# carlosnatalino/optical-rl-gym

Measured on NVIDIA B200. Metric: env_steps_per_sec, higher is better.
Workload: dtype u32

## Files before the change

### optical-rl-gym_b200/csrc/orlg_api.cu

```cuda
#include <atomic>
#include <cmath>
#include <condition_variable>
#include <cstdio>
#include <cstdlib>
#include <chrono>
#include <cstring>
#include <emmintrin.h>
#include <functional>
#include <memory>
#include <mutex>
#include <string>
#include <thread>
#include <vector>

#include "orlg_deeprmsa_fast.cuh"
#include "orlg_rollout.cuh"
#include "orlg_policy.cuh"
#include "orlg_step_wide.cuh"
#include "orlg_wrappers.cuh"

using namespace orlg;

static thread_local std::string g_err;

// ... 364 lines not shown
    p.seed = cfg->seed; p.env_id_base = cfg->env_id_base;
    p.mean_holding = cfg->mean_holding; p.mean_iat = cfg->mean_iat;
    p.obs_dim = cfg->kind == ORLG_DEEPRMSA ? 1 + 2 * p.N + (2 * J + 3) * p.k : 0;
    p.node_top_step = 1;
    while (p.node_top_step * 2 <= p.N - 1) p.node_top_step *= 2;
    p.cand_stride = ((p.k * J + 7) / 8) * 8;
    p.nwv = wide ? (p.S + 127) / 128 : 1;
    p.wstride = wide ? (p.nwv == 3 ? 4 : p.nwv) : 0;
    env->km = p.k <= 5 ? 5 : KMAX;
    env->obs_smem = (size_t)STEP_THREADS * p.obs_dim * (p.obs_f64 ? 8 : 4);
    if (env->obs_smem > 200 * 1024) { delete env; return fail(ORLG_E_UNSUPPORTED, "observation too large for the staging tile"); }

    int cap = cfg->heap_capacity;
    if (cap <= 0) {
        double load = cfg->mean_holding / cfg->mean_iat;
        double want = load + 8.0 * std::sqrt(load) + 16.0;
        double hard = cfg->kind == ORLG_RWA ? (double)p.E * p.S * C : (double)p.E * p.S * C / 2.0;
        cap = (int)std::ceil(want < hard ? want : hard);
    }
    cap = ((cap + EV_GROUP - 1) / EV_GROUP) * EV_GROUP;
    if (cfg->heap_capacity > 256 * EV_GROUP) {
        delete env;
        return fail(ORLG_E_UNSUPPORTED, "heap_capacity above 4096 live services per environment");
    }
    if (cap > 256 * EV_GROUP) cap = 256 * EV_GROUP;
    p.ev_groups = ((cap / EV_GROUP + 15) / 16) * 16;
    p.heap_cap = cap;

    int rc = ORLG_OK;
    const int NN = p.N * p.N, P = t->num_paths;
    std::vector<int> pair_first(t->pair_first, t->pair_first + NN);
    std::vector<unsigned char> pair_count(NN);
    for (int i = 0; i < NN; i++) pair_count[i] = (unsigned char)(t->pair_count[i] < 0 ? 0 : (t->pair_count[i] > p.k ? p.k : t->pair_count[i]));
    std::vector<unsigned> linkmask(P), meta(P);
    int se_max = 1;
    for (int r = 0; r < P; r++) {
        unsigned lm = 0;
        for (int h = t->path_link_ptr[r]; h < t->path_link_ptr[r + 1]; h++) {
            if (t->path_links[h] < 0 || t->path_links[h] >= p.E) { delete env; return fail(ORLG_E_INVALID, "path link index out of range"); }
            if (!wide) lm |= 1u << t->path_links[h];
        }
        if (t->path_hops[r] > 255 || t->path_link_ptr[r + 1] - t->path_link_ptr[r] != t->path_hops[r]) { delete env; return fail(ORLG_E_INVALID, "inconsistent path hop counts"); }
        linkmask[r] = lm;
        int se = t->path_se[r] < 1 ? 1 : t->path_se[r];
        meta[r] = (unsigned)(t->path_hops[r] & 0xff) | ((unsigned)(se & 0xff) << 8) | ((unsigned)(t->path_mod[r] & 0xff) << 16);
        se_max = se > se_max ? se : se_max;
    }
    std::vector<unsigned char> mod_se(t->num_mods > 0 ? t->num_mods : 1, 1);
    for (int m = 0; m < t->num_mods; m++) { mod_se[m] = (unsigned char)t->mod_se[m]; se_max = t->mod_se[m] > se_max ? t->mod_se[m] : se_max; }
    std::vector<unsigned char> nslots((size_t)(se_max + 1) * (br_max + 1), 1);
    bool slots_unrepresentable = false;
    for (int se = 1; se <= se_max; se++)
        for (int b = 0; b <= br_max; b++) {
            int n = (int)std::ceil((double)b / ((double)se * cfg->channel_width)) + 1;
            if (n > 200) {
                const bool configured = t->num_bit_rates > 0 ? false : (b >= cfg->bit_rate_lo && b <= cfg->bit_rate_hi);
                if (n <= p.S && configured) slots_unrepresentable = true;
                n = 200;
            }
            nslots[(size_t)se * (br_max + 1) + b] = (unsigned char)n;
        }
    for (int i = 0; i < t->num_bit_rates; i++)
        for (int se = 1; se <= se_max; se++) {
            const int n = (int)std::ceil((double)t->bit_rates[i] / ((double)se * cfg->channel_width)) + 1;
            if (n > 200 && n <= p.S) slots_unrepresentable = true;
        }
    if (slots_unrepresentable && cfg->kind != ORLG_RWA) {
        delete env;
        return fail(ORLG_E_UNSUPPORTED, "a request of this configuration may need 201.." + std::to_string(p.S) + " slots: at most 200 slots per service are representable");
    }
    std::vector<double> reach((size_t)(t->num_mods > 0 ? t->num_mods : 1) * (br_max + 1), 0.0);
    if (cfg->kind == ORLG_RMCSA)
        for (int m = 0; m < t->num_mods; m++)
            for (int b = 0; b <= br_max; b++)
                reach[(size_t)m * (br_max + 1) + b] = b == 0 ? 1e300 : reach_km(t->mod_osnr[m], t->mod_xt[m], t->mod_se[m], b, cfg->worst_xt);
    std::vector<double> plen(t->path_length, t->path_length + P);
    std::vector<unsigned> node_thr = thresholds(t->node_prob, p.N);
    std::vector<unsigned> br_thr = t->num_bit_rates > 0 ? thresholds(t->bit_rate_prob, t->num_bit_rates) : std::vector<unsigned>(1, 0u);
    std::vector<int> link_order(p.E);
    for (int l = 0; l < p.E; l++) link_order[l] = t->link_order ? t->link_order[l] : l;
    std::vector<int> bit_rates(t->num_bit_rates > 0 ? t->num_bit_rates : 1, 0);
    for (int i = 0; i < t->num_bit_rates; i++) bit_rates[i] = t->bit_rates[i];

    if (!rc) rc = dev_upload(env, &p.pair_first, pair_first);
    if (!rc) rc = dev_upload(env, &p.pair_count, pair_count);
    if (!rc) rc = dev_upload(env, &p.path_linkmask, linkmask);
    if (!rc) rc = dev_upload(env, &p.path_meta, meta);
    if (!rc) rc = dev_upload(env, &p.path_length, plen);
    {
        std::vector<int> lptr(t->path_link_ptr, t->path_link_ptr + P + 1);
        std::vector<unsigned short> l16(lptr[P] > 0 ? lptr[P] : 1, 0);
        for (int h = 0; h < lptr[P]; h++) l16[h] = (unsigned short)t->path_links[h];
        if (!rc) rc = dev_upload(env, &p.path_link_ptr, lptr);
        if (!rc) rc = dev_upload(env, &p.path_links16, l16);
    }
    if (!rc) rc = dev_upload(env, &p.nslots, nslots);
    if (!rc) rc = dev_upload(env, &p.mod_se, mod_se);
    if (!rc) rc = dev_upload(env, &p.reach, reach);
    if (!rc) rc = dev_upload(env, &p.node_thr, node_thr);
    if (!rc) rc = dev_upload(env, &p.br_thr, br_thr);
    if (!rc) rc = dev_upload(env, &p.bit_rates, bit_rates);
    if (!rc) rc = dev_upload(env, &p.link_order, link_order);
    env->alloc_is_state = true;
    const size_t n = (size_t)p.n;
    if (!rc) rc = dev_alloc(env, &p.masks, (size_t)C * p.E * (wide ? p.wstride : p.nwv) * n);
    if (!rc) rc = dev_alloc(env, &p.now, n);
    if (!rc) rc = dev_alloc(env, &p.cur_hold, n);
    if (!rc) rc = dev_alloc(env, &p.cur_req, n);
    if (!rc) rc = dev_alloc(env, &p.counters, 8 * n);
    if (!rc) rc = dev_alloc(env, &p.req_index, n);
    if (!rc) rc = dev_alloc(env, &p.nheap, n);
    if (!rc) rc = dev_alloc(env, &p.heap_min, n);
    if (!rc) rc = dev_alloc(env, &p.ev_time, n * (size_t)p.heap_cap, false);
    if (!rc) rc = dev_alloc(env, &p.ev_pay, n * (size_t)p.heap_cap, false);
    if (!rc) rc = dev_alloc(env, &p.ev_gmin, n * (size_t)p.ev_groups);
    if (!rc) rc = dev_alloc(env, &p.ev_tail, n);
    if (!rc) rc = dev_alloc(env, &p.cand, n * (size_t)p.cand_stride);
    if (!rc && wide && cfg->kind == ORLG_DEEPRMSA) rc = dev_alloc(env, &p.cand16, n * (size_t)p.cand_stride);
    if (!rc) rc = dev_alloc(env, &p.errors, n);
    if (!rc && cfg->kind == ORLG_RMSA && t->num_bit_rates > 0) rc = dev_alloc(env, &p.br_hist, 2 * (size_t)t->num_bit_rates * n);
    if (!rc && cfg->kind == ORLG_RWA) rc = dev_alloc(env, &p.act_hist, (size_t)(p.k + p.S + 2 * p.allow_rejection) * n);
    env->alloc_is_state = false;
    if (rc) { orlg_destroy(env); return rc; }

    env->fast = false;
    env->hot = false;
    env->ro_ok = false;
    if (!wide && cfg->kind != ORLG_RMCSA && p.k <= 5 && P <= 65535 && se_max <= 15 && !std::getenv("ORLG_FORCE_GENERIC")) {
        std::vector<unsigned char> blob;
        auto put = [&blob](const void *src, size_t bytes) {
            size_t off = (blob.size() + 15) / 16 * 16;
            blob.resize(off + bytes);
            std::memcpy(blob.data() + off, src, bytes);
            return (int)off;
        };
        std::vector<unsigned short> pf16(NN);
        for (int i = 0; i < NN; i++) pf16[i] = (unsigned short)(pair_first[i] < 0 ? 0 : pair_first[i]);
        std::vector<unsigned char> pse(P);
        for (int r = 0; r < P; r++) pse[r] = (unsigned char)((meta[r] >> 8) & 0xff);
        std::vector<unsigned char> ns128((size_t)(se_max + 1) * 128, 1);
        for (int se = 1; se <= se_max; se++)
            for (int b = 0; b < 128 && b <= br_max; b++) ns128[(size_t)se * 128 + b] = nslots[(size_t)se * (br_max + 1) + b];
        std::vector<float> pos(p.S + 1), nsl(32);
        for (int v = 0; v <= p.S; v++) pos[v] = (float)(2 * v - p.S) / (float)p.S;
        for (int v = 0; v < 32; v++) nsl[v] = (float)(2 * v - 11) / 7.0f;
        p.off_pair_first = put(pf16.data(), pf16.size() * 2);
        p.off_pair_count = put(pair_count.data(), pair_count.size());
        p.off_path_lm = put(linkmask.data(), linkmask.size() * 4);
        p.off_path_se = put(pse.data(), pse.size());
        std::vector<unsigned long long> pll(P, 0ULL);
        bool ll_ok = true;
        for (int r = 0; r < P; r++) {
            const int h0 = t->path_link_ptr[r], hn = t->path_link_ptr[r + 1] - h0;
            if (hn > 12) { ll_ok = false; break; }
            unsigned long long v = (unsigned long long)hn << 60;
            for (int h = 0; h < hn; h++) v |= (unsigned long long)(t->path_links[h0 + h] & 31) << (5 * h);
            pll[r] = v;
        }
        p.off_path_ll = put(pll.data(), pll.size() * 8);
        p.off_nslots = put(ns128.data(), ns128.size());
        p.off_node_thr = put(node_thr.data(), node_thr.size() * 4);
        p.off_pos = put(pos.data(), pos.size() * 4);
        p.off_nsl = put(nsl.data(), nsl.size() * 4);
        std::vector<float> rcp4(p.S / 2 + 2, 0.0f);
        for (size_t r = 1; r < rcp4.size(); r++) rcp4[r] = 1.0f / (float)(4 * r);
        p.off_rcp4 = put(rcp4.data(), rcp4.size() * 4);
        std::vector<unsigned> dbl(17, 0u);
        for (int nn = 1; nn <= 16; nn++) {
            int len = 1;
            for (int it = 0; it < 4; it++) {
                int sh = len < nn - len ? len : nn - len;
                if (sh < 0) sh = 0;
                dbl[nn] |= (unsigned)sh << (8 * it);
                len += sh;
            }
        }
        p.off_dbl = put(dbl.data(), dbl.size() * 4);
        blob.resize((blob.size() + 127) / 128 * 128);
        if (ll_ok && blob.size() <= 24 * 1024 && blob.size() + (size_t)FAST_THREADS * 16 * 32 <= 100 * 1024) {
            std::vector<uint4> blob4(blob.size() / 16);
            std::memcpy(blob4.data(), blob.data(), blob.size());
            rc = dev_upload(env, &p.tab_blob, blob4);
            if (rc) { orlg_destroy(env); return rc; }
            p.tab_vec = (int)blob4.size();
            env->fast = cfg->kind == ORLG_DEEPRMSA;
            size_t per_thread = (size_t)p.obs_dim * (p.obs_f64 ? 8 : 4);
            if (per_thread < (size_t)p.E * 16) per_thread = (size_t)p.E * 16;
            p.warp_area_bytes = (int)((per_thread * 32 + 127) / 128 * 128);
            env->fast_smem = blob.size() + (size_t)(FAST_THREADS / 32) * p.warp_area_bytes + 8 * (FAST_THREADS / 32 + 1);
            cudaError_t ea = cudaSuccess;
            if (env->fast_smem > 48 * 1024) {
                ea = cudaFuncSetAttribute(deeprmsa_fast_kernel<22, 5, 1, false>, cudaFuncAttributeMaxDynamicSharedMemorySize, (int)env->fast_smem);
                if (ea == cudaSuccess) ea = cudaFuncSetAttribute(deeprmsa_fast_kernel<0, 5, 1, false>, cudaFuncAttributeMaxDynamicSharedMemorySize, (int)env->fast_smem);
                if (ea == cudaSuccess) ea = cudaFuncSetAttribute(deeprmsa_fast_kernel<22, 5, 1, true>, cudaFuncAttributeMaxDynamicSharedMemorySize, (int)env->fast_smem);
                if (ea == cudaSuccess) ea = cudaFuncSetAttribute(deeprmsa_fast_kernel<0, 5, 1, true>, cudaFuncAttributeMaxDynamicSharedMemorySize, (int)env->fast_smem);
                if (ea == cudaSuccess) ea = cudaFuncSetAttribute(deeprmsa_fast_kernel<22, 5, 0, false>, cudaFuncAttributeMaxDynamicSharedMemorySize, (int)env->fast_smem);
                if (ea == cudaSuccess) ea = cudaFuncSetAttribute(deeprmsa_fast_kernel<0, 5, 0, false>, cudaFuncAttributeMaxDynamicSharedMemorySize, (int)env->fast_smem);
                if (ea == cudaSuccess) ea = cudaFuncSetAttribute(deeprmsa_fast_kernel<22, 5, 0, true>, cudaFuncAttributeMaxDynamicSharedMemorySize, (int)env->fast_smem);
                if (ea == cudaSuccess) ea = cudaFuncSetAttribute(deeprmsa_fast_kernel<0, 5, 0, true>, cudaFuncAttributeMaxDynamicSharedMemorySize, (int)env->fast_smem);
            }
            if (ea == cudaSuccess && env->fast_smem > 48 * 1024) {
                ea = cudaFuncSetAttribute(deeprmsa_fast_kernel<22, 5, 1, false, true>, cudaFuncAttributeMaxDynamicSharedMemorySize, (int)env->fast_smem);
                if (ea == cudaSuccess) ea = cudaFuncSetAttribute(deeprmsa_fast_kernel<0, 5, 1, false, true>, cudaFuncAttributeMaxDynamicSharedMemorySize, (int)env->fast_smem);
            }
            if (ea != cudaSuccess) env->fast = false;
            int n_hi = 0;
            for (int se = 1; se <= se_max; se++)
                for (int b = 0; b <= cfg->bit_rate_hi && b <= br_max; b++)
                    n_hi = nslots[(size_t)se * (br_max + 1) + b] > n_hi ? nslots[(size_t)se * (br_max + 1) + b] : n_hi;
            env->hot = env->fast && J == 1 && p.k == 5 && p.cand_stride == 8 && t->num_bit_rates == 0 && cfg->bit_rate_hi < 128 &&
                       cfg->bit_rate_lo >= 0 && n_hi <= 16 && (p.obs_dim & 1) == 0 && p.E <= 256 && !std::getenv("ORLG_NO_HOT");
            if (env->hot && !encode_mask_map(env)) env->hot = false;
            const bool small_n = t->num_bit_rates == 0 && cfg->bit_rate_hi < 128 && cfg->bit_rate_lo >= 0 && n_hi <= 16;
            env->ro_ok = cfg->kind == ORLG_DEEPRMSA ? env->hot
                         : (ea == cudaSuccess && p.E <= 32 && (cfg->kind == ORLG_RWA || small_n) && !std::getenv("ORLG_NO_HOT"));
        }
    }

    if (env->obs_smem > 48 * 1024) {
        cudaError_t e1 = cudaFuncSetAttribute(step_kernel<ORLG_DEEPRMSA, 5>, cudaFuncAttributeMaxDynamicSharedMemorySize, (int)env->obs_smem);
        cudaError_t e2 = cudaFuncSetAttribute(step_kernel<ORLG_DEEPRMSA, KMAX>, cudaFuncAttributeMaxDynamicSharedMemorySize, (int)env->obs_smem);
        if (e1 != cudaSuccess || e2 != cudaSuccess) { orlg_destroy(env); return fail(ORLG_E_CUDA, "cudaFuncSetAttribute(shared memory) failed"); }
    }
    *out = env;
    return ORLG_OK;
}

int orlg_destroy(orlg_env *env) {
    if (!env) return ORLG_OK;
    DeviceGuard guard(env->device);
    for (void *ptr : env->allocs) cudaFree(ptr);
    for (int i = 0; i < RO_HOST_BUFFERS; i++) {
        if (env->ro_pk_dev[i]) cudaFree(env->ro_pk_dev[i]);
        if (env->ro_pk_host[i]) cudaFreeHost(env->ro_pk_host[i]);
        if (env->ro_pk_ev[i]) cudaEventDestroy(env->ro_pk_ev[i]);
        if (env->ro_k_ev[i]) cudaEventDestroy(env->ro_k_ev[i]);
        if (env->ro_act_dev[i]) cudaFree(env->ro_act_dev[i]);
        if (env->ro_obs_dev[i]) cudaFree(env->ro_obs_dev[i]);
        if (env->ro_cp_ev[i]) cudaEventDestroy(env->ro_cp_ev[i]);
    }
    if (env->ro_copy_stream) cudaStreamDestroy(env->ro_copy_stream);
    delete env;
    return ORLG_OK;
}

int orlg_action_dim(const orlg_env *env) { return env->p.kind == ORLG_DEEPRMSA ? 1 : (env->p.kind == ORLG_RMCSA ? 4 : 2); }
int orlg_obs_dim(const orlg_env *env) { return env->p.obs_dim; }
int orlg_mask_words(const orlg_env *env) { return NW * env->p.nwv; }
int orlg_heap_capacity(const orlg_env *env) { return env->p.heap_cap; }
int64_t orlg_state_bytes(const orlg_env *env) { return env->state_bytes; }

int orlg_kernel_info(const orlg_env *env, orlg_kernel_info_t *out) {
    if (!env || !out) return fail(ORLG_E_INVALID, "null handle or output");
    out->wide = env->wide;
    out->fast = env->fast;
    out->hot = env->hot;
    out->rollout_kernel = env->ro_ok;
    out->rollout_lanes = rollout_lpw(env);
    out->link_template = !env->wide && env->p.E == 22 ? 22 : 0;
    out->last_rollout_persistent = env->ro_last_persistent;
    return ORLG_OK;
}

int orlg_seed(orlg_env *env, uint64_t seed) {
    if (!env) return fail(ORLG_E_INVALID, "null handle");
    env->p.seed = seed;
    env->cfg.seed = seed;
    return ORLG_OK;
}

int orlg_set_trace(orlg_env *env, const orlg_request *trace_dev, int64_t trace_len) {
    if (!env || (trace_len > 0 && !trace_dev)) return fail(ORLG_E_INVALID, "null trace");
    if (trace_len >= (1LL << 32)) return fail(ORLG_E_UNSUPPORTED, "trace too long");
    env->p.trace = trace_dev;
    env->p.trace_len = trace_len;
    env->p.traffic = ORLG_TRAFFIC_TRACE;
    return ORLG_OK;
}

int orlg_reset(orlg_env *env, int full, void *obs_dev, orlg_stream stream) {
    if (!env) return fail(ORLG_E_INVALID, "null handle");
    DeviceGuard guard(env->device);
    if (env->p.traffic == ORLG_TRAFFIC_TRACE && env->p.trace == nullptr) return fail(ORLG_E_INVALID, "trace traffic selected but orlg_set_trace was not called");
    StepIO io;
    std::memset(&io, 0, sizeof(io));
    io.policy = -1;
    io.obs = env->p.obs_dim ? obs_dev : nullptr;
    if (full) env->ro_valid = false;
    else {
        int rc0 = ensure_canonical(env, (cudaStream_t)stream);
        if (rc0) return rc0;
    }
    if (full) {
        fill_events_kernel<<<592, 256, 0, (cudaStream_t)stream>>>(env->p);
        CUDA_OK(cudaGetLastError());
    }
    int rc = launch_step(env, io, full ? MODE_FULL_RESET : MODE_EPISODE_RESET, (cudaStream_t)stream);
    if (rc == ORLG_OK && full) env->p.lockstep_ridx = 1;
    return rc;
}

static int step_impl(orlg_env *env, const int32_t *actions_dev, int fused_policy, int32_t *actions_out, void *obs_dev, float *reward_dev,
                     uint8_t *done_dev, int32_t *decision_dev, int64_t *info_dev, orlg_stream stream) {
    {
        int rc0 = ensure_canonical(env, (cudaStream_t)stream);
        if (rc0) return rc0;
    }
    StepIO io;
    io.policy = fused_policy;
// ... 861 lines not shown
```

### optical-rl-gym_b200/csrc/orlg_rollout.cuh

```cuda
#pragma once
#include "orlg_deeprmsa_fast.cuh"

#ifndef ORLG_RO_BULK
#define ORLG_RO_BULK 1
#endif

namespace orlg {

constexpr int RO_WCAP = 64;
#ifndef ORLG_RO_SIDE
#define ORLG_RO_SIDE 4
#endif
constexpr int RO_SIDE = ORLG_RO_SIDE;
constexpr int RO_MAX_THREADS = 448;
enum { RO_POLICY_RANDOM = 0, RO_POLICY_SP_FF = 1, RO_POLICY_SAP_FF = 2, RO_POLICY_REPLAY = 3, RO_POLICY_LLP_FF = 4, RO_POLICY_SAP_LF = 5 };

#ifdef ORLG_PHASE_TIMING
#define RPH_INIT() long long rph_t_ = clock64()
#define RPH_MARK(k)                                                                                      \
    do {                                                                                                 \
        long long rph_n_ = clock64();                                                                    \
        if ((threadIdx.x & 31) == 0) atomicAdd(&g_phase_cycles[k], (unsigned long long)(rph_n_ - rph_t_)); \
        rph_t_ = rph_n_;                                                                                 \
    } while (0)
// ... 439 lines not shown
                if (POLICY == RO_POLICY_SP_FF) {
                    if (npaths_cur > 0 && (candw & 0xffu) != CAND_NONE) { act = 0; act_slot = (int)(candw & 0xffu); }
                } else if (POLICY == RO_POLICY_LLP_FF) {
                    int best = KIND == ORLG_RWA ? -1 : 0;
                    for (int q = 0; q < npaths_cur; q++) {
                        const unsigned st = (unsigned)((candw >> (8 * q)) & 0xffu);
                        const int fr = (int)((candt >> (8 * q)) & 0xffu);
                        if (st != CAND_NONE && fr > best) { best = fr; act = q; act_slot = (int)st; }
                    }
                } else if (KIND == ORLG_RWA) {
                    int best_hops = 0x7fffffff;
                    for (int q = 0; q < npaths_cur; q++) {
                        const unsigned st = (unsigned)((candw >> (8 * q)) & 0xffu);
                        const int hops = (int)((candh >> (4 * q)) & 0xfu);
                        if (hops < best_hops && st != CAND_NONE) { best_hops = hops; act = q; act_slot = (int)st; }
                    }
                } else {
                    for (int q = npaths_cur - 1; q >= 0; q--) {
                        const unsigned st = (unsigned)((candw >> (8 * q)) & 0xffu);
                        if (st != CAND_NONE) { act = q; act_slot = (int)st; }
                    }
                }
            }
            if (POLICY != RO_POLICY_REPLAY && ra.actions) {
                if (KIND == ORLG_DEEPRMSA) ra.actions[(size_t)t * p.n + env] = act;
                else *reinterpret_cast<int2 *>(ra.actions + ((size_t)t * p.n + env) * 2) = make_int2(act, act_slot);
            }

            bool accepted = false;
            int a_start = 0;
            if (KIND == ORLG_RWA && p.act_hist) {
                const int R = p.k + p.allow_rejection, Cn = p.S + p.allow_rejection;
                if (act >= 0 && act < R && act_slot >= 0 && act_slot < Cn) {
                    atomicAdd(p.act_hist + (size_t)act * p.n + env, 1);
                    atomicAdd(p.act_hist + (size_t)(R + act_slot) * p.n + env, 1);
                } else {
                    err |= ORLG_ERR_NO_SUCH_PATH;
                }
            }
            if (act >= 0 && act < p.k && (KIND == ORLG_DEEPRMSA || (act_slot >= 0 && act_slot < p.S))) {
                if (act < np_cur) {
                    const int a_row = s_pair_first[pair] + act;
                    const int a_n = KIND == ORLG_RWA ? 1 : s_nslots[s_path_se[a_row] * 128 + br];
                    const unsigned a_lm = s_path_lm[a_row];
                    bool fits;
                    if (KIND == ORLG_DEEPRMSA) {
                        const unsigned st = (unsigned)((candw >> (8 * act)) & 0xffu);
                        fits = st != CAND_NONE;
                        a_start = (int)st;
                    } else if (checked) {
                        fits = true; a_start = act_slot;
                    } else {
                        a_start = act_slot;
                        fits = a_start + a_n <= p.S;
                        if (fits) {
                            Bits F = bits_ones();
                            unsigned m = a_lm;
                            while (m) {
                                const int l = __ffs(m) - 1;
                                m &= m - 1;
                                F = bits_and(F, bits_from(sm[l * 32]));
                            }
                            fits = bits_contains(F, bits_range_short(a_start, a_n));
                        }
                    }
                    if (fits) {
                        if (nlive + 1 > (unsigned)p.heap_cap) {
                            err |= ORLG_ERR_HEAP_OVERFLOW;
                        } else {
                            ro_path_update<false>(sm, a_lm, bits_range_short(a_start, a_n));
                            const double rel = __dadd_rn(now, hold);
                            const unsigned long long pl = pack_service(a_row, a_start, a_n, 0, sid);
                            bool in_side = false;
                            if (rel <= hzn) {
#pragma unroll
                                for (int s = 0; s < RO_SIDE; s++) {
                                    if (!in_side && !(side_t[s * 32] < ORLG_INF)) {
                                        side_t[s * 32] = rel; side_p[s * 32] = pl; in_side = true;
                                    }
                                }
                                if (in_side) side_min = dmin(side_min, rel);
                            }
                            if (!in_side) {
                                win_store(ev + n_tab * 32, rel, pl); n_tab++;
                                tmin_tab = dmin(tmin_tab, rel);
                            }
                            nlive++;
                            d_acc += 1; ep_acc += 1;
                            if (KIND != ORLG_RWA) { d_prov += br; ep_prov += br; }
                            accepted = true;
                        }
                    }
                } else {
                    err |= ORLG_ERR_NO_SUCH_PATH;
                }
            }
            if (KIND == ORLG_RWA) { d_proc += 1; ep_proc += 1; }
            if (ra.reward) ra.reward[(size_t)t * p.n + env] = accepted ? 1.0f : (KIND == ORLG_DEEPRMSA ? -1.0f : 0.0f);
            rec_flags = ((unsigned)act & 0xffffu) | (accepted ? (1u << 28) : 0u);

            RPH_MARK(1);
            now = TRACE ? t_arrival : __dadd_rn(now, e_iat);
            hold = e_hold; src = p_src; dst = p_dst; br = p_br;
            ridx++;
            sid = ep_proc;
            if (KIND != ORLG_RWA) { d_proc += 1; ep_proc += 1; d_req += br; ep_req += br; }
            npaths_cur = npaths;
            RO_POP_DUE();
            if (side_min <= now) {
                double m2 = ORLG_INF;
#pragma unroll
                for (int s = 0; s < RO_SIDE; s++) {
                    const double ts = side_t[s * 32];
                    if (ts <= now) {
                        const unsigned long long pl = side_p[s * 32];
                        const int rs = svc_start(pl);
                        ro_path_update<true>(sm, s_path_lm[svc_row(pl)], bits_range_short(rs, svc_slots(pl)));
                        side_t[s * 32] = ORLG_INF;
                        nlive--;
                    } else {
                        m2 = dmin(m2, ts);
                    }
                }
                side_min = m2;
            }
        }
        RPH_MARK(2);
        for (int tries = 0; t >= 0 && __any_sync(0xffffffffu, live && tmin_tab <= now); tries++) {
            RPH_COUNT(15);
            hzn = tries < 60 ? __dadd_rn(now, __dmul_rn(ra.span, __longlong_as_double((long long)(1023 - tries) << 52))) : now;
            RTL_REBUILD_BEGIN();
            unsigned long long g_rtl_scan_ = 0, g_rtl_sort_ = 0;
            ro_rebuild(ev, (unsigned)p.heap_cap, side_t, side_p, n_tab, wh, wn, tmin_tab, side_min, hzn, head, nxt, lane, g_rtl_scan_, g_rtl_sort_);
            RO_POP_DUE();
            RTL_REBUILD_END();
        }
        RPH_MARK(3);
        if (live && t >= 0) {
            done = (ep_proc == p.episode_length);
            if (done && p.auto_reset) {
                ep_acc = 0; ep_prov = 0;
                if (KIND == ORLG_RWA) { ep_proc = 0; ep_req = 0; } else { ep_proc = 1; ep_req = br; }
            }
            if (ra.done) ra.done[(size_t)t * p.n + env] = done ? 1 : 0;
        }

        unsigned feat[KM];
#pragma unroll
        for (int q = 0; q < KM; q++) feat[q] = 0;
        if (live) {
            unsigned long long cand_out = 0xFFFFFFFFFFFFFFFFULL, tot_out = 0;
            unsigned hops_out = 0;
            const int first = s_pair_first[src * p.N + dst];
#pragma unroll 1
            for (int q = 0; q < KM; q++) {
                const bool have = q < npaths;
                const int row = have ? first + q : first;
                unsigned lm = have ? s_path_lm[row] : 0u;
                Bits A = have ? bits_ones() : Bits{{0u, 0u, 0u, 0u}};
                while (lm) {
                    const int l0 = __ffs(lm) - 1;
                    lm &= lm - 1;
                    const int l1 = lm ? __ffs(lm) - 1 : l0;
                    lm &= lm - 1;
                    const int l2 = lm ? __ffs(lm) - 1 : l0;
                    lm &= lm - 1;
                    const int l3 = lm ? __ffs(lm) - 1 : l0;
                    lm &= lm - 1;
                    const uint4 v0 = sm[l0 * 32], v1 = sm[l1 * 32], v2 = sm[l2 * 32], v3 = sm[l3 * 32];
                    A.w[0] &= v0.x & v1.x; A.w[1] &= v0.y & v1.y; A.w[2] &= v0.z & v1.z; A.w[3] &= v0.w & v1.w;
                    A.w[0] &= v2.x & v3.x; A.w[1] &= v2.y & v3.y; A.w[2] &= v2.z & v3.z; A.w[3] &= v2.w & v3.w;
                }
                int st;
                unsigned f = 0;
                if (KIND == ORLG_DEEPRMSA) {
                    const int n = s_nslots[s_path_se[row] * 128 + br];
                    const Bits B = bits_runs_ge_sched(A, s_dbl[n]);
                    st = bits_ffs_flat(B);
                    const int fe = bits_ffs_flat(bits_andnot(B, bits_shr1(B)));
                    const int total = bits_popc(A);
                    const int runs = bits_popc(bits_andnot(A, bits_shl1(A)));
                    f = feat_pack(st, fe - st + n, total, runs, n);
                } else {
                    if (KIND == ORLG_RWA) {
                        if (POLICY == RO_POLICY_SAP_LF) { Bits L = A; L.w[0] &= ~1u; st = bits_fls(L); }
                        else st = bits_ffs_flat(A);
                        if (have) hops_out |= (unsigned)(s_path_ll[row] >> 60) << (4 * q);
                    } else {
                        const int n = s_nslots[s_path_se[row] * 128 + br];
                        const Bits B = bits_and(bits_runs_ge_sched(A, s_dbl[n]), bits_range(0, max(p.S - n, 0)));
                        st = bits_ffs_flat(B);
                    }
                    tot_out |= (unsigned long long)(bits_popc(A) & 0xff) << (8 * q);
                }
                cand_out = st >= 0 ? ((cand_out & ~(0xFFULL << (8 * q))) | ((unsigned long long)st << (8 * q))) : cand_out;
#pragma unroll
                for (int i = 0; i < KM; i++) feat[i] = i == q ? f : feat[i];
            }
            if (KIND != ORLG_DEEPRMSA) { candt = tot_out; candh = hops_out; }
            candw = cand_out;
        }
        RPH_MARK(5);
        if (t < 0) continue;
        if (KIND == ORLG_DEEPRMSA && ra.packed && live) {
            uint4 *rec = ra.packed + ((size_t)t * p.n + env) * 2;
            rec[0] = make_uint4(feat[0], feat[1], feat[2], feat[3]);
            rec[1] = make_uint4(feat[4], (unsigned)br | ((unsigned)src << 8) | ((unsigned)dst << 16) | ((unsigned)npaths << 24) |
                                             (rec_flags & (1u << 28)) | (done ? (1u << 29) : 0u),
                                rec_flags & 0xffffu, 0u);
        }
        if (KIND == ORLG_DEEPRMSA && ra.obs) {
            const unsigned tile = ro_tile_acquire(pool_free, lane);
            unsigned char *stage = pool + (size_t)tile * ra.tile_bytes;
            RPH_MARK(4);
            if (live) {
                float *so32 = reinterpret_cast<float *>(stage) + (size_t)lane * p.obs_dim;
                float2 *r2 = reinterpret_cast<float2 *>(so32);
                const int lo_n = min(src, dst), hi_n = max(src, dst);
                for (int q = 0; q < p.N; q++) r2[q] = make_float2(0.0f, 0.0f);
                float v[2 + 5 * KM];
                v[0] = hi_n == p.N - 1 ? 1.0f : 0.0f;
                v[1 + 5 * KM] = 0.0f;
#pragma unroll
                for (int q = 0; q < KM; q++) {
                    const unsigned f = feat[q];
                    const int st = (int)(f & 127u), len = (int)((f >> 7) & 127u), total = (int)((f >> 14) & 127u);
                    const int runs = (int)((f >> 21) & 63u), n = (int)(f >> 27);
                    const bool have = q < npaths, blk = st != 127;
                    v[1 + 5 * q] = blk ? s_pos[blk ? st : 0] : -1.0f;
                    v[2 + 5 * q] = blk ? (float)(len - 8) * 0.125f : -1.0f;
                    v[3 + 5 * q] = have ? s_nsl[n] : -1.0f;
                    v[4 + 5 * q] = have ? s_pos[total] : -1.0f;
                    v[5 + 5 * q] = runs > 0 ? (float)(total - 4 * runs) * s_rcp4[runs] : -1.0f;
                }
#pragma unroll
                for (int i = 0; i < (1 + 5 * KM + 1) / 2; i++) r2[p.N + i] = make_float2(v[2 * i], v[2 * i + 1]);
                so32[0] = __fdiv_rn((float)br, 100.0f);
                so32[1 + lo_n] = 1.0f;
                if (hi_n != p.N - 1) so32[1 + p.N + hi_n] = 1.0f;
            }
            RPH_MARK(6);
            {
                float *g = ra.obs + ((size_t)t * p.n + env0) * p.obs_dim;
                const int total_el = nvalid * p.obs_dim;
#if ORLG_RO_BULK
                asm volatile("fence.proxy.async.shared::cta;" ::: "memory");
                __syncwarp();
                if ((reinterpret_cast<size_t>(g) & 15) == 0 && (total_el & 3) == 0) {
                    if (lane == 0) {
                        asm volatile("cp.async.bulk.global.shared::cta.bulk_group [%0], [%1], %2;"
                                     ::"l"(g), "r"((unsigned)__cvta_generic_to_shared(stage)), "r"((unsigned)total_el * 4u) : "memory");
                        asm volatile("cp.async.bulk.commit_group;" ::: "memory");
                        asm volatile("cp.async.bulk.wait_group.read 0;" ::: "memory");
                    }
                } else {
                    const float *sv = reinterpret_cast<const float *>(stage);
                    for (int q = lane; q < total_el; q += 32) g[q] = sv[q];
                }
#else
                __syncwarp();
                if ((reinterpret_cast<size_t>(g) & 15) == 0 && (total_el & 3) == 0) {
                    const uint4 *sv = reinterpret_cast<const uint4 *>(stage);
                    uint4 *gv = reinterpret_cast<uint4 *>(g);
#pragma unroll 7
                    for (int q = lane; q < total_el / 4; q += 32) gv[q] = sv[q];
                } else {
                    const float *sv = reinterpret_cast<const float *>(stage);
                    for (int q = lane; q < total_el; q += 32) g[q] = sv[q];
                }
#endif
            }
            ro_tile_release(pool_free, tile, lane);
        }
        RPH_MARK(7);
    }
#undef RO_POP_DUE
    RTL_SET(2);

    if (live) {
        ra.st_ntab[env] = n_tab; ra.st_wh[env] = wh; ra.st_wn[env] = wn;
        ra.st_tmin[env] = tmin_tab; ra.st_hzn[env] = hzn;
#pragma unroll
        for (int s = 0; s < RO_SIDE; s++) {
            ra.st_side_t[(size_t)s * p.n + env] = side_t[s * 32];
            ra.st_side_p[(size_t)s * p.n + env] = side_p[s * 32];
        }
        uint4 *mw = p.masks + env;
        for (int l = 0; l < E; l++) mw[(size_t)l * p.n] = sm[l * 32];
        p.now[env] = now;
        p.cur_hold[env] = hold;
        p.cur_req[env] = make_uint2((unsigned)src | ((unsigned)dst << 8) | ((unsigned)br << 16), (unsigned)sid);
        {
            const auto c0 = p.counters[(size_t)0 * p.n + env], c1 = p.counters[(size_t)1 * p.n + env];
            const auto c4 = p.counters[(size_t)4 * p.n + env], c5 = p.counters[(size_t)5 * p.n + env];
            p.counters[(size_t)0 * p.n + env] = c0 + d_proc;
            p.counters[(size_t)1 * p.n + env] = c1 + d_acc;
            p.counters[(size_t)4 * p.n + env] = c4 + d_req;
            p.counters[(size_t)5 * p.n + env] = c5 + d_prov;
        }
        p.counters[(size_t)2 * p.n + env] = ep_proc;
        p.counters[(size_t)3 * p.n + env] = ep_acc;
        p.counters[(size_t)6 * p.n + env] = ep_req;
        p.counters[(size_t)7 * p.n + env] = ep_prov;
        p.req_index[env] = ridx;
        p.nheap[env] = nlive;
        p.errors[env] = err;
        if (KIND == ORLG_DEEPRMSA) *reinterpret_cast<unsigned long long *>(p.cand + (size_t)env * 8) = candw;
    }
    RPH_MARK(9);
    RTL_SET(3);
    RTL_FLUSH((unsigned)gwarp);
}

__global__ void __launch_bounds__(128) ro_canonicalize_kernel(const Params p, const RolloutArgs ra) {
    const int env = blockIdx.x * blockDim.x + threadIdx.x;
    if (env >= p.n) return;
    const int lane = env % ra.lpw;
    const size_t gw = (size_t)(env / ra.lpw);
    WinEntry *const ev = ra.ev + gw * (size_t)(p.heap_cap + 2 * RO_WCAP) * 32 + lane;
    const WinEntry *const win = ev + (size_t)(p.heap_cap + RO_WCAP) * 32;
    unsigned n_tab = ra.st_ntab[env];
    const unsigned wh = ra.st_wh[env], wn = ra.st_wn[env], n_entry = ra.st_ncanon[env];
    unsigned err = 0;
    for (unsigned j = wh; j < wn; j++) {
        const WinEntry w = win_load(win + j * 32);
        win_store(ev + n_tab * 32, w.t, w.p); n_tab++;
    }
#pragma unroll
    for (int s = 0; s < RO_SIDE; s++) {
        const double ts = ra.st_side_t[(size_t)s * p.n + env];
        if (ts < ORLG_INF) { win_store(ev + n_tab * 32, ts, ra.st_side_p[(size_t)s * p.n + env]); n_tab++; }
    }
    if (n_tab != p.nheap[env]) err |= ORLG_ERR_LOCKSTEP;
    double *ev_t = p.ev_time + (size_t)env * p.heap_cap;
    unsigned long long *ev_p = p.ev_pay + (size_t)env * p.heap_cap;
    float *gmin = p.ev_gmin + (size_t)env * p.ev_groups;
    const unsigned n_fill = max(n_tab, n_entry);
    for (unsigned s0 = 0; s0 < n_fill; s0 += 8) {
        double tt[8];
        unsigned long long pp[8];
#pragma unroll
        for (int i = 0; i < 8; i++) {
            const bool in = s0 + i < n_tab;
            WinEntry w;
            w.t = ORLG_INF; w.p = 0ULL;
            if (in) w = win_load(ev + (s0 + i) * 32);
            tt[i] = w.t; pp[i] = w.p;
        }
#pragma unroll
        for (int i = 0; i < 4; i++) {
// ... 24 lines not shown
```

Before: 5.981 billion.

## Walk packed per-path link lists instead of bitmask ffs loop; pair paths for RMSA/RWA

Candidate scoring now reads each path's links from a packed 64-bit list (hop count plus 5-bit link ids) instead of pulling links out of a 32-bit mask with repeated ffs. Host packing pads unused slots with the first link, so four-link chunks can read past the hop count without changing the AND result. The non-DeepRMSA branch handles two paths per iteration to expose more independent shared-memory loads. Risks: paths with zero hops, or more than 12, now mark the packing invalid, and the kernel branch may not check that flag. The paired loop also runs to the longer path's hop count.

Result: faster. 6.275 billion (median of 6 runs) (+4.9%).

```diff
diff --git a/optical-rl-gym_b200/csrc/orlg_api.cu b/optical-rl-gym_b200/csrc/orlg_api.cu
--- a/optical-rl-gym_b200/csrc/orlg_api.cu
+++ b/optical-rl-gym_b200/csrc/orlg_api.cu
@@ -540,9 +540,9 @@
         bool ll_ok = true;
         for (int r = 0; r < P; r++) {
             const int h0 = t->path_link_ptr[r], hn = t->path_link_ptr[r + 1] - h0;
-            if (hn > 12) { ll_ok = false; break; }
+            if (hn > 12 || hn < 1) { ll_ok = false; break; }
             unsigned long long v = (unsigned long long)hn << 60;
-            for (int h = 0; h < hn; h++) v |= (unsigned long long)(t->path_links[h0 + h] & 31) << (5 * h);
+            for (int h = 0; h < 12; h++) v |= (unsigned long long)(t->path_links[h0 + (h < hn ? h : 0)] & 31) << (5 * h);
             pll[r] = v;
         }
         p.off_path_ll = put(pll.data(), pll.size() * 8);
diff --git a/optical-rl-gym_b200/csrc/orlg_rollout.cuh b/optical-rl-gym_b200/csrc/orlg_rollout.cuh
--- a/optical-rl-gym_b200/csrc/orlg_rollout.cuh
+++ b/optical-rl-gym_b200/csrc/orlg_rollout.cuh
@@ -615,50 +615,86 @@
             unsigned long long cand_out = 0xFFFFFFFFFFFFFFFFULL, tot_out = 0;
             unsigned hops_out = 0;
             const int first = s_pair_first[src * p.N + dst];
+            if (KIND == ORLG_DEEPRMSA) {
 #pragma unroll 1
-            for (int q = 0; q < KM; q++) {
-                const bool have = q < npaths;
-                const int row = have ? first + q : first;
-                unsigned lm = have ? s_path_lm[row] : 0u;
-                Bits A = have ? bits_ones() : Bits{{0u, 0u, 0u, 0u}};
-                while (lm) {
-                    const int l0 = __ffs(lm) - 1;
-                    lm &= lm - 1;
-                    const int l1 = lm ? __ffs(lm) - 1 : l0;
-                    lm &= lm - 1;
-                    const int l2 = lm ? __ffs(lm) - 1 : l0;
-                    lm &= lm - 1;
-                    const int l3 = lm ? __ffs(lm) - 1 : l0;
-                    lm &= lm - 1;
-                    const uint4 v0 = sm[l0 * 32], v1 = sm[l1 * 32], v2 = sm[l2 * 32], v3 = sm[l3 * 32];
-                    A.w[0] &= v0.x & v1.x; A.w[1] &= v0.y & v1.y; A.w[2] &= v0.z & v1.z; A.w[3] &= v0.w & v1.w;
-                    A.w[0] &= v2.x & v3.x; A.w[1] &= v2.y & v3.y; A.w[2] &= v2.z & v3.z; A.w[3] &= v2.w & v3.w;
-                }
-                int st;
-                unsigned f = 0;
-                if (KIND == ORLG_DEEPRMSA) {
+                for (int q = 0; q < KM; q++) {
+                    const bool have = q < npaths;
+                    const int row = have ? first + q : first;
+                    unsigned long long ll = s_path_ll[row];
                     const int n = s_nslots[s_path_se[row] * 128 + br];
-                    const Bits B = bits_runs_ge_sched(A, s_dbl[n]);
-                    st = bits_ffs_flat(B);
+                    const unsigned sched = s_dbl[n];
+                    Bits A = have ? bits_ones() : Bits{{0u, 0u, 0u, 0u}};
+                    for (int h = have ? (int)(ll >> 60) : 0; h > 0; h -= 4, ll >>= 20) {
+                        const unsigned w = (unsigned)ll;
+                        const uint4 v0 = sm[(w & 31u) * 32], v1 = sm[((w >> 5) & 31u) * 32];
+                        const uint4 v2 = sm[((w >> 10) & 31u) * 32], v3 = sm[((w >> 15) & 31u) * 32];
+                        A.w[0] &= v0.x & v1.x; A.w[1] &= v0.y & v1.y; A.w[2] &= v0.z & v1.z; A.w[3] &= v0.w & v1.w;
+                        A.w[0] &= v2.x & v3.x; A.w[1] &= v2.y & v3.y; A.w[2] &= v2.z & v3.z; A.w[3] &= v2.w & v3.w;
+                    }
+                    RPH_MARK(10);
+                    const Bits B = bits_runs_ge_sched(A, sched);
+                    const int st = bits_ffs_flat(B);
                     const int fe = bits_ffs_flat(bits_andnot(B, bits_shr1(B)));
                     const int total = bits_popc(A);
                     const int runs = bits_popc(bits_andnot(A, bits_shl1(A)));
-                    f = feat_pack(st, fe - st + n, total, runs, n);
-                } else {
-                    if (KIND == ORLG_RWA) {
-                        if (POLICY == RO_POLICY_SAP_LF) { Bits L = A; L.w[0] &= ~1u; st = bits_fls(L); }
-                        else st = bits_ffs_flat(A);
-                        if (have) hops_out |= (unsigned)(s_path_ll[row] >> 60) << (4 * q);
-                    } else {
-                        const int n = s_nslots[s_path_se[row] * 128 + br];
-                        const Bits B = bits_and(bits_runs_ge_sched(A, s_dbl[n]), bits_range(0, max(p.S - n, 0)));
-                        st = bits_ffs_flat(B);
-                    }
-                    tot_out |= (unsigned long long)(bits_popc(A) & 0xff) << (8 * q);
-                }
-                cand_out = st >= 0 ? ((cand_out & ~(0xFFULL << (8 * q))) | ((unsigned long long)st << (8 * q))) : cand_out;
-#pragma unroll
-                for (int i = 0; i < KM; i++) feat[i] = i == q ? f : feat[i];
+                    const unsigned f = feat_pack(st, fe - st + n, total, runs, n);
+                    cand_out = st >= 0 ? ((cand_out & ~(0xFFULL << (8 * q))) | ((unsigned long long)st << (8 * q))) : cand_out;
+#pragma unroll
+                    for (int i = 0; i < KM; i++) feat[i] = i == q ? f : feat[i];
+                    RPH_MARK(5);
+                }
+            } else {
+#pragma unroll 1
+                for (int q = 0; q < KM; q += 2) {
+                    bool have[2];
+                    int row[2], n[2] = {0, 0};
+                    unsigned sched[2] = {0u, 0u};
+                    unsigned long long ll[2];
+                    Bits A[2];
+#pragma unroll
+                    for (int j = 0; j < 2; j++) {
+                        have[j] = q + j < npaths;
+                        row[j] = have[j] ? first + q + j : first;
+                        ll[j] = s_path_ll[row[j]];
+                        if (KIND != ORLG_RWA) {
+                            n[j] = s_nslots[s_path_se[row[j]] * 128 + br];
+                            sched[j] = s_dbl[n[j]];
+                        }
+                        A[j] = have[j] ? bits_ones() : Bits{{0u, 0u, 0u, 0u}};
+                    }
+                    const int hops = max(have[0] ? (int)(ll[0] >> 60) : 0, have[1] ? (int)(ll[1] >> 60) : 0);
+                    for (int s = 0; s < 5 * hops; s += 10) {
+                        uint4 v[2][2];
+#pragma unroll
+                        for (int j = 0; j < 2; j++)
+#pragma unroll
+                            for (int h = 0; h < 2; h++) v[j][h] = sm[(int)((ll[j] >> (s + 5 * h)) & 31u) * 32];
+#pragma unroll
+                        for (int j = 0; j < 2; j++) {
+                            A[j].w[0] &= v[j][0].x & v[j][1].x;
+                            A[j].w[1] &= v[j][0].y & v[j][1].y;
+                            A[j].w[2] &= v[j][0].z & v[j][1].z;
+                            A[j].w[3] &= v[j][0].w & v[j][1].w;
+                        }
+                    }
+                    RPH_MARK(10);
+#pragma unroll
+                    for (int j = 0; j < 2; j++) {
+                        const int qj = q + j;
+                        int st;
+                        if (KIND == ORLG_RWA) {
+                            if (POLICY == RO_POLICY_SAP_LF) { Bits L = A[j]; L.w[0] &= ~1u; st = bits_fls(L); }
+                            else st = bits_ffs_flat(A[j]);
+                            if (have[j]) hops_out |= (unsigned)(ll[j] >> 60) << (4 * qj);
+                        } else {
+                            const Bits B = bits_and(bits_runs_ge_sched(A[j], sched[j]), bits_range(0, max(p.S - n[j], 0)));
+                            st = bits_ffs_flat(B);
+                        }
+                        tot_out |= (unsigned long long)(bits_popc(A[j]) & 0xff) << (8 * qj);
+                        cand_out = st >= 0 ? ((cand_out & ~(0xFFULL << (8 * qj))) | ((unsigned long long)st << (8 * qj))) : cand_out;
+                    }
+                    RPH_MARK(5);
+                }
             }
             if (KIND != ORLG_DEEPRMSA) { candt = tot_out; candh = hops_out; }
             candw = cand_out;
```
